# broadinstitute/permutect

Measured on AMD Instinct MI355X. Metric: read-sets/sec (train fwd+bwd), higher is better.
Workload: dtype f32 (fp32 accumulate; fwd: 2 x f16 pieces per operand = 23 bits; bwd: 2 x bf16 pieces = 16 bits)

## Files before the change

### include/permutect_amd.h

```cpp
#ifndef PERMUTECT_AMD_H
#define PERMUTECT_AMD_H

#include <stddef.h>
#include <stdint.h>

#ifdef __cplusplus
extern "C" {
#endif

#define PMT_ABI_VERSION 11

#define PMT_FAULT_JOIN 1
#define PMT_FAULT_F16_RANGE 2
#define PMT_FAULT_PLAN 4

#define PMT_OK 0
#define PMT_E_INVALID (-1)
#define PMT_E_UNSUPPORTED (-2)
#define PMT_E_CAPACITY (-3)
#define PMT_E_LAUNCH (-4)
#define PMT_E_WORKSPACE (-5)

#ifndef PMT_MAX_WIDTH
#define PMT_MAX_WIDTH 64
#endif
// ... 192 lines not shown
#define PMT_PHI_LOG_SOFTMAX 3
#define PMT_PHI_ORTHOGONAL 4
#define PMT_MAX_PHI_SEGS 48
#define PMT_MAX_ORTHO_DIM 32
typedef struct PmtPhiSeg {
    int32_t kind, theta_off, phi_off, rows, cols, reserved;
    float p0, p1;
    int32_t base_rs, base_cs;
    const float* base;
} PmtPhiSeg;
typedef struct PmtPhiProgram {
    int32_t n_segs, reserved;
    PmtPhiSeg seg[PMT_MAX_PHI_SEGS];
} PmtPhiProgram;

int pmt_phi_forward(const PmtPhiProgram* prog, const float* theta, float* phi, void* stream);
int pmt_phi_backward(const PmtPhiProgram* prog, const float* theta, const float* phi, const float* grad_phi,
                     float* grad_theta, void* stream);

typedef struct PmtIntColumn {
    const void* ptr;
    int64_t stride;
    int32_t elem_bytes, reserved;
} PmtIntColumn;

typedef struct PmtBinning {
    int32_t num_sources, num_variant_types, num_ref_bins, num_alt_bins, count_bin_skip, max_ref_count, max_alt_count, reserved;
} PmtBinning;

typedef struct PmtDownsample {
    int32_t num_variants;
// ... 32 lines not shown
    const int64_t* labels;
    int64_t label_stride;
    const int64_t* alt_counts;
    int64_t alt_count_stride;
    const int64_t* sources;
    int64_t source_stride;
    const float* weights;
    const float* source_weights;
} PmtLossArgs;
typedef struct PmtLossOutputs {
    float* supervised_b;
    float* unsupervised_b;
    float* alt_count_b;
    float* source_b;
    float* total_b;
} PmtLossOutputs;
typedef struct PmtLossInputGrads {
    float* d_logits_b;
    float* d_logits_bk;
    float* d_alt_count_raw;
    float* d_source_logits;
} PmtLossInputGrads;
int pmt_losses_forward(const PmtLossArgs* args, const PmtLossOutputs* out, void* stream);
int pmt_losses_backward(const PmtLossArgs* args, const PmtLossOutputs* grad_out, const PmtLossInputGrads* grad_in, void* stream);

typedef struct PmtRecordArgs {
    int32_t num_variants, num_bins;
    int32_t num_variant_types, num_ref_bins, num_alt_bins, count_bin_skip, max_ref_count, max_alt_count;
    PmtIntColumn labels, variant_types, sources, ref_counts, alt_counts;
    const float* weights;
// ... 136 lines not shown
```

### permutect_amd/architecture/artifact_model.py

```python
from __future__ import annotations

from typing import Optional

import torch
from torch import Tensor, nn

from permutect_amd import constants
from permutect_amd.architecture import modules as M
from permutect_amd.data.batch import Batch
from permutect_amd.data.datum import Data
from permutect_amd.engine import lib as L
from permutect_amd.engine.runtime import (HaplotypeCnnFunction, LossesFunction, PhiFunction, ReadSetEngine, ReadSetFunction,
                                          RowsMlpFunction, VariantEmbedFunction)
from permutect_amd.enums import Epoch
from permutect_amd.parameters import ModelParameters, install_pickle_alias

_BCE = nn.BCEWithLogitsLoss(reduction="none")


def gpu_if_available() -> torch.device:
    return torch.device("cuda" if torch.cuda.is_available() else "cpu")


class BatchOutput:

    def __init__(self, features_be: Tensor, ref_features_be: Tensor, logits_b: Tensor, logits_bk: Tensor,
                 weights: Tensor, source_weights: Tensor):
        self.features_be = features_be
        self.ref_features_be = ref_features_be
        self.logits_b = logits_b
        self.logits_bk = logits_bk
        self.weights = weights
        self.source_weights = source_weights

    @property
    def artifact_probs_b(self) -> Tensor:
        return torch.sigmoid(self.logits_b)

    @property
    def outlier_binary_logits(self) -> Tensor:
        lk = self.logits_bk
        nonoutlier = torch.logsumexp(torch.cat((lk[:, 0:1], lk[:, 2:]), dim=-1), dim=-1)
        return lk[:, 1] - nonoutlier


class BatchLosses:

    def __init__(self, supervised_losses_b, unsupervised_losses_b, alt_count_losses_b, source_prediction_losses_b,
                 total_losses_b):
        self.supervised_losses_b = supervised_losses_b
        self.unsupervised_losses_b = unsupervised_losses_b
        self.alt_count_losses_b = alt_count_losses_b
        self.source_prediction_losses_b = source_prediction_losses_b
        self.total_losses_b = total_losses_b
        self.total_loss = torch.sum(total_losses_b)


class SetMeansView:

    def __init__(self, means_be: Tensor, lengths_b: Tensor):
        self._means, self.lengths_b = means_be, lengths_b

    def means_over_sets(self) -> Tensor:
        return self._means

    def batch_size(self) -> int:
        return len(self.lengths_b)


class ArtifactModel(nn.Module):
# ... 97 lines not shown
            eng.pack(phi.detach().contiguous())
            eng.packed_for = (key, phi.detach()) if (key is not None and not torch.is_grad_enabled()) else None
        variant_embed = self.variant_embedding(batch)
        outs = ReadSetFunction.apply(eng, batch, phi, variant_embed)
        return outs, variant_embed

    def calculate_features(self, batch: Batch, weight_range: float = 0):
        (logits_b, logits_bk, feats, ref_feats), ve = self._encode(batch)
        e_hap = self.haplotypes_cnn.output_dimension()
        return (SetMeansView(ref_feats, batch.get(Data.REF_COUNT)), SetMeansView(feats, batch.get(Data.ALT_COUNT)),
                ve[:, ve.shape[1] - e_hap:])

    def compute_batch_output(self, batch: Batch, balancer=None) -> BatchOutput:
        (logits_b, logits_bk, feats, ref_feats), _ = self._encode(batch)
        if balancer is None:
            weights_b = source_weights = torch.ones_like(logits_b)
        elif logits_b.is_cuda and hasattr(balancer, "weights_from_logits"):
            weights_b, source_weights = balancer.weights_from_logits(batch, logits_b)
        else:
            weights_b, source_weights_b = balancer.process_batch_and_compute_weights(
                batch, artifact_probs_b=torch.sigmoid(logits_b).detach())
            source_weights = weights_b * source_weights_b
        return BatchOutput(features_be=feats, ref_features_be=ref_feats, logits_b=logits_b, logits_bk=logits_bk,
                           weights=weights_b, source_weights=source_weights)

    def compute_source_prediction_losses(self, features_be: Tensor, batch: Batch) -> Tensor:
        if self.num_sources > 1:
            eng = self.engine()
            logits = RowsMlpFunction.apply(eng, L.ROWS_SOURCE, features_be, eng.trigger,
                                           float(self.source_predictor.gradient_reversal.alpha))
            probs = torch.softmax(logits, dim=-1)
# ... 6 lines not shown
        raw = RowsMlpFunction.apply(eng, L.ROWS_ALT_COUNT, features_be, eng.trigger,
                                    float(self.alt_count_predictor.gradient_reversal.alpha))
        pred = torch.sigmoid(raw.view(-1))
        target = batch.get(Data.ALT_COUNT).to(dtype=pred.dtype) / constants.MAX_ALT_COUNT
        return self.alt_count_loss_func(pred, target)

    def compute_batch_losses(self, output: BatchOutput, batch: Batch) -> BatchLosses:
        eng = self.engine()
        alt_raw = RowsMlpFunction.apply(eng, L.ROWS_ALT_COUNT, output.features_be, eng.trigger,
                                        float(self.alt_count_predictor.gradient_reversal.alpha))
        source_logits, sources = None, None
        if self.num_sources > 1:
            source_logits = RowsMlpFunction.apply(eng, L.ROWS_SOURCE, output.features_be, eng.trigger,
                                                  float(self.source_predictor.gradient_reversal.alpha))
            sources = batch.get(Data.SOURCE).long()
        sup, unsup, alt, src, total = LossesFunction.apply(
            eng, output.logits_b, output.logits_bk, alt_raw, source_logits, batch.get(Data.LABEL).long(),
            batch.get(Data.ALT_COUNT).long(), sources, output.weights, output.source_weights)
        return BatchLosses(sup, unsup, alt, src, total)

    def compute_batch_losses_torch(self, output: BatchOutput, batch: Batch) -> BatchLosses:
        labels_b = batch.get_training_labels()
        is_labeled_b = batch.get_is_labeled_mask()
        supervised = is_labeled_b * _BCE(output.logits_b, labels_b)
        clipped = torch.clip(output.outlier_binary_logits, max=constants.MAX_OUTLIER_LOGIT)
        unsupervised = (1 - is_labeled_b) * _BCE(clipped, torch.zeros_like(clipped))
        alt_count = self.compute_alt_count_losses(output.features_be, batch)
        source = self.compute_source_prediction_losses(output.features_be, batch)
        total = output.weights * (supervised + unsupervised + alt_count) + output.source_weights * source
        return BatchLosses(supervised, unsupervised, alt_count, source, total)

    def make_dict_for_saving(self, artifact_log_priors=None, artifact_spectra=None):
        state = {k: v.detach().clone() for k, v in self.state_dict().items()}
        return {
# ... 28 lines not shown
```

### permutect_amd/csrc/pmt_losses.hip

```cpp
#include <hip/hip_runtime.h>
#include <math.h>

#include "permutect_amd.h"

#define LOSS_THREADS 256

__device__ __forceinline__ float softplus_f(float x) { return fmaxf(x, 0.f) + log1pf(expf(-fabsf(x))); }
__device__ __forceinline__ float sigmoid_f(float x) { return 1.0f / (1.0f + expf(-x)); }

struct OutlierLogit {
    float o;
    float mx, se;
};
__device__ __forceinline__ OutlierLogit outlier_logit(const float* __restrict__ lk, int K) {
    OutlierLogit r;
    r.mx = lk[0];
    for (int k = 0; k < K; ++k) r.mx = fmaxf(r.mx, lk[2 + k]);
    r.se = expf(lk[0] - r.mx);
    for (int k = 0; k < K; ++k) r.se += expf(lk[2 + k] - r.mx);
    r.o = lk[1] - (r.mx + logf(r.se));
    return r;
}

__global__ __launch_bounds__(LOSS_THREADS) void pmt_losses_forward_kernel(PmtLossArgs a, PmtLossOutputs out) {
    const int b = blockIdx.x * LOSS_THREADS + threadIdx.x;
    if (b >= a.num_variants) return;
    const int K = a.num_clusters, S = a.num_sources;
    const long long label = a.labels[(size_t)b * a.label_stride];
    const float is_labeled = label != 2 ? 1.f : 0.f;
    const float target = label == 0 ? 1.f : (label == 2 ? 0.5f : 0.f);
    const float x = a.logits_b[b];
    const float sup = is_labeled * (fmaxf(x, 0.f) - x * target + log1pf(expf(-fabsf(x))));
    const OutlierLogit ol = outlier_logit(a.logits_bk + (size_t)b * (K + 2), K);
    const float unsup = (1.f - is_labeled) * softplus_f(fminf(ol.o, a.max_outlier_logit));
    const float pred = sigmoid_f(a.alt_count_raw[b]);
    const float tgt = (float)a.alt_counts[(size_t)b * a.alt_count_stride] / a.max_alt_count;
    const float altl = (pred - tgt) * (pred - tgt);
    float src = 0.f;
    if (S > 1 && a.source_logits != nullptr) {
        const float* sl = a.source_logits + (size_t)b * S;
        const long long sid = a.sources[(size_t)b * a.source_stride];
        float mx = sl[0];
        for (int s = 1; s < S; ++s) mx = fmaxf(mx, sl[s]);
        float se = 0.f;
        for (int s = 0; s < S; ++s) se += expf(sl[s] - mx);
        for (int s = 0; s < S; ++s) {
            const float d = expf(sl[s] - mx) / se - (s == sid ? 1.f : 0.f);
            src += d * d;
        }
    }
    out.supervised_b[b] = sup;
    out.unsupervised_b[b] = unsup;
    out.alt_count_b[b] = altl;
    out.source_b[b] = src;
    out.total_b[b] = a.weights[b] * (sup + unsup + altl) + a.source_weights[b] * src;
}

__global__ __launch_bounds__(LOSS_THREADS) void pmt_losses_backward_kernel(PmtLossArgs a, PmtLossOutputs g, PmtLossInputGrads d) {
    const int b = blockIdx.x * LOSS_THREADS + threadIdx.x;
    if (b >= a.num_variants) return;
    const int K = a.num_clusters, S = a.num_sources;
    const float gt = g.total_b ? g.total_b[b] : 0.f;
    const float g_sup = (g.supervised_b ? g.supervised_b[b] : 0.f) + gt * a.weights[b];
    const float g_unsup = (g.unsupervised_b ? g.unsupervised_b[b] : 0.f) + gt * a.weights[b];
    const float g_alt = (g.alt_count_b ? g.alt_count_b[b] : 0.f) + gt * a.weights[b];
    const float g_src = (g.source_b ? g.source_b[b] : 0.f) + gt * a.source_weights[b];
    const long long label = a.labels[(size_t)b * a.label_stride];
    const float is_labeled = label != 2 ? 1.f : 0.f;
    const float target = label == 0 ? 1.f : (label == 2 ? 0.5f : 0.f);
    d.d_logits_b[b] = g_sup * is_labeled * (sigmoid_f(a.logits_b[b]) - target);
    const float* lk = a.logits_bk + (size_t)b * (K + 2);
    float* dlk = d.d_logits_bk + (size_t)b * (K + 2);
    const OutlierLogit ol = outlier_logit(lk, K);
    const float go = ol.o <= a.max_outlier_logit ? g_unsup * (1.f - is_labeled) * sigmoid_f(ol.o) : 0.f;
    dlk[1] = go;
    dlk[0] = -go * expf(lk[0] - ol.mx) / ol.se;
    for (int k = 0; k < K; ++k) dlk[2 + k] = -go * expf(lk[2 + k] - ol.mx) / ol.se;
    const float pred = sigmoid_f(a.alt_count_raw[b]);
    const float tgt = (float)a.alt_counts[(size_t)b * a.alt_count_stride] / a.max_alt_count;
    d.d_alt_count_raw[b] = g_alt * 2.f * (pred - tgt) * pred * (1.f - pred);
    if (S > 1 && a.source_logits != nullptr && d.d_source_logits != nullptr) {
// ... 7 lines not shown
        float dot = 0.f;
        for (int s = 0; s < S; ++s) {
            const float p = expf(sl[s] - mx) / se;
            dot += 2.f * (p - (s == sid ? 1.f : 0.f)) * p;
        }
        for (int s = 0; s < S; ++s) {
            const float p = expf(sl[s] - mx) / se;
            dsl[s] = g_src * (2.f * (p - (s == sid ? 1.f : 0.f)) * p - p * dot);
        }
    }
}

static int loss_args_check(const PmtLossArgs* a) {
    if (!a || a->num_variants < 0 || a->num_clusters < 0 || a->num_clusters > PMT_MAX_CLUSTERS || a->num_sources < 1) return PMT_E_INVALID;
    if (a->num_variants == 0) return PMT_OK;
    if (!a->logits_b || !a->logits_bk || !a->alt_count_raw || !a->labels || !a->alt_counts || !a->weights || !a->source_weights)
        return PMT_E_INVALID;
    if (a->num_sources > 1 && a->source_logits && !a->sources) return PMT_E_INVALID;
    return PMT_OK;
}

extern "C" int pmt_losses_forward(const PmtLossArgs* args, const PmtLossOutputs* out, void* stream) {
    const int rc = loss_args_check(args);
    if (rc) return rc;
    if (!out || !out->supervised_b || !out->unsupervised_b || !out->alt_count_b || !out->source_b || !out->total_b) return PMT_E_INVALID;
    if (args->num_variants == 0) return PMT_OK;
    hipLaunchKernelGGL(pmt_losses_forward_kernel, dim3((args->num_variants + LOSS_THREADS - 1) / LOSS_THREADS), dim3(LOSS_THREADS), 0,
                       reinterpret_cast<hipStream_t>(stream), *args, *out);
    return hipGetLastError() == hipSuccess ? PMT_OK : PMT_E_LAUNCH;
}

extern "C" int pmt_losses_backward(const PmtLossArgs* args, const PmtLossOutputs* grad_out, const PmtLossInputGrads* grad_in,
                                   void* stream) {
    const int rc = loss_args_check(args);
    if (rc) return rc;
    if (!grad_out || !grad_in || !grad_in->d_logits_b || !grad_in->d_logits_bk || !grad_in->d_alt_count_raw) return PMT_E_INVALID;
    if (args->num_variants == 0) return PMT_OK;
    hipLaunchKernelGGL(pmt_losses_backward_kernel, dim3((args->num_variants + LOSS_THREADS - 1) / LOSS_THREADS), dim3(LOSS_THREADS), 0,
                       reinterpret_cast<hipStream_t>(stream), *args, *grad_out, *grad_in);
    return hipGetLastError() == hipSuccess ? PMT_OK : PMT_E_LAUNCH;
}
// ... 89 lines not shown
```

### permutect_amd/csrc/pmt_phi.hip

```cpp
#include <hip/hip_runtime.h>
#include <math.h>

#include "permutect_amd.h"

#define PHI_THREADS 256
#define PHI_MAXN (2 * PMT_MAX_ORTHO_DIM)

__device__ double block_max(double v, double* red) {
    const int tid = threadIdx.x;
    red[tid] = v;
    __syncthreads();
    for (int s = PHI_THREADS / 2; s > 0; s >>= 1) {
        if (tid < s) red[tid] = fmax(red[tid], red[tid + s]);
        __syncthreads();
    }
    const double r = red[0];
    __syncthreads();
    return r;
}
__device__ double block_sum(double v, double* red) {
    const int tid = threadIdx.x;
    red[tid] = v;
    __syncthreads();
    for (int s = PHI_THREADS / 2; s > 0; s >>= 1) {
        if (tid < s) red[tid] += red[tid + s];
        __syncthreads();
    }
    const double r = red[0];
    __syncthreads();
    return r;
}

__device__ void matmul(double* __restrict__ Cm, const double* __restrict__ A, const double* __restrict__ B, int N, double scale) {
    for (int idx = threadIdx.x; idx < N * N; idx += PHI_THREADS) {
        const int i = idx / N, j = idx - i * N;
        double a0 = 0.0, a1 = 0.0, a2 = 0.0, a3 = 0.0;
        const double* ar = A + i * N;
        const double* bc = B + j;
        int k = 0;
        for (; k + 3 < N; k += 4) {
            a0 += ar[k] * bc[k * N];
            a1 += ar[k + 1] * bc[(k + 1) * N];
            a2 += ar[k + 2] * bc[(k + 2) * N];
            a3 += ar[k + 3] * bc[(k + 3) * N];
        }
        for (; k < N; ++k) a0 += ar[k] * bc[k * N];
        Cm[idx] = ((a0 + a1) + (a2 + a3)) * scale;
    }
    __syncthreads();
}

__device__ void expm_inplace(double* S, double* B, double* P, double* T, int N, double* red) {
    double colsum = 0.0;
    if (threadIdx.x < N)
        for (int i = 0; i < N; ++i) colsum += fabs(S[i * N + threadIdx.x]);
    const double norm1 = block_max(colsum, red);
    int s = 0;
    if (norm1 > 0.5) s = (int)ceil(log2(norm1 / 0.5));
    const double scale = ldexp(1.0, -s);
    for (int idx = threadIdx.x; idx < N * N; idx += PHI_THREADS) {
        const double b = S[idx] * scale;
        B[idx] = b;
        P[idx] = b;
        const int i = idx / N, j = idx - i * N;
        S[idx] = b + (i == j ? 1.0 : 0.0);
    }
    __syncthreads();
    for (int k = 2; k <= 12; ++k) {
        matmul(T, P, B, N, 1.0 / (double)k);
        for (int idx = threadIdx.x; idx < N * N; idx += PHI_THREADS) {
            P[idx] = T[idx];
            S[idx] += T[idx];
        }
        __syncthreads();
    }
    for (int q = 0; q < s; ++q) {
        matmul(T, S, S, N, 1.0);
        for (int idx = threadIdx.x; idx < N * N; idx += PHI_THREADS) S[idx] = T[idx];
        __syncthreads();
    }
}

struct PhiShared {
    double m[4][PHI_MAXN * PHI_MAXN];
    double red[PHI_THREADS];
};
static_assert(sizeof(PhiShared) <= 160 * 1024, "LDS budget");

__global__ __launch_bounds__(PHI_THREADS) void pmt_phi_forward_kernel(PmtPhiProgram prog, const float* __restrict__ theta,
                                                                       float* __restrict__ phi) {
    __shared__ __attribute__((aligned(16))) PhiShared sh;
    const PmtPhiSeg sg = prog.seg[blockIdx.x];
    const float* x = theta + sg.theta_off;
    float* y = phi + sg.phi_off;
    const int tid = threadIdx.x, n = sg.rows * sg.cols;
    if (sg.kind == PMT_PHI_EXP) {
        for (int i = tid; i < n; i += PHI_THREADS) y[i] = expf(x[i]);
    } else if (sg.kind == PMT_PHI_BOUNDED) {
        for (int i = tid; i < n; i += PHI_THREADS) y[i] = sg.p1 * (1.0f / (1.0f + expf(-x[i]))) + sg.p0;
    } else if (sg.kind == PMT_PHI_UNIT_ROWS) {
        for (int r = 0; r < sg.rows; ++r) {
            double q = 0.0;
            for (int i = tid; i < sg.cols; i += PHI_THREADS) q += (double)x[r * sg.cols + i] * (double)x[r * sg.cols + i];
            const float norm = (float)sqrt(block_sum(q, sh.red));
            for (int i = tid; i < sg.cols; i += PHI_THREADS) y[r * sg.cols + i] = x[r * sg.cols + i] / norm;
        }
    } else if (sg.kind == PMT_PHI_LOG_SOFTMAX) {
        for (int r = 0; r < sg.rows; ++r) {
            double mx = -INFINITY;
            for (int i = tid; i < sg.cols; i += PHI_THREADS) mx = fmax(mx, (double)x[r * sg.cols + i]);
            mx = block_max(mx, sh.red);
            double se = 0.0;
            for (int i = tid; i < sg.cols; i += PHI_THREADS) se += exp((double)x[r * sg.cols + i] - mx);
            const double lse = mx + log(block_sum(se, sh.red));
            for (int i = tid; i < sg.cols; i += PHI_THREADS) y[r * sg.cols + i] = (float)((double)x[r * sg.cols + i] - lse);
        }
    } else if (sg.kind == PMT_PHI_ORTHOGONAL) {
        const int N = sg.rows;
        double* S = sh.m[0];
        for (int idx = tid; idx < N * N; idx += PHI_THREADS) {
            const int i = idx / N, j = idx - i * N;
            S[idx] = i > j ? (double)x[i * N + j] : (i < j ? -(double)x[j * N + i] : 0.0);
        }
        __syncthreads();
        expm_inplace(S, sh.m[1], sh.m[2], sh.m[3], N, sh.red);
        for (int idx = tid; idx < N * N; idx += PHI_THREADS) {
            const int i = idx / N, j = idx - i * N;
            double acc = 0.0;
            if (sg.base != nullptr) {
                for (int k = 0; k < N; ++k) acc += (double)sg.base[i * sg.base_rs + k * sg.base_cs] * S[k * N + j];
            } else {
                acc = S[idx];
            }
            y[idx] = (float)acc;
        }
    }
}

__global__ __launch_bounds__(PHI_THREADS) void pmt_phi_backward_kernel(PmtPhiProgram prog, const float* __restrict__ theta,
                                                                        const float* __restrict__ phi,
                                                                        const float* __restrict__ gphi,
                                                                        float* __restrict__ gtheta) {
    __shared__ __attribute__((aligned(16))) PhiShared sh;
    const PmtPhiSeg sg = prog.seg[blockIdx.x];
    const float* x = theta + sg.theta_off;
    const float* y = phi + sg.phi_off;
    const float* gy = gphi + sg.phi_off;
// ... 41 lines not shown
            G[idx] = acc;
        }
        __syncthreads();
        for (int idx = tid; idx < N * N; idx += PHI_THREADS) {
            const int i = idx / N, j = idx - i * N;
            const int bi = i % nn, bj = j % nn;
            double v = 0.0;
            if ((i < nn) == (j < nn)) {
                v = bi > bj ? -(double)x[bi * nn + bj] : (bi < bj ? (double)x[bj * nn + bi] : 0.0);
            } else if (i < nn) {
                v = G[bi * nn + bj];
            }
            S[idx] = v;
        }
        __syncthreads();
        double* B = sh.m[1];
        expm_inplace(S, B, sh.m[2], sh.m[3], N, sh.red);
        for (int idx = tid; idx < nn * nn; idx += PHI_THREADS) {
            const int i = idx / nn, j = idx - i * nn;
            if (i > j) gx[idx] += (float)(S[i * N + nn + j] - S[j * N + nn + i]);
        }
    }
}

static int phi_check(const PmtPhiProgram* p) {
    if (!p || p->n_segs < 0 || p->n_segs > PMT_MAX_PHI_SEGS) return PMT_E_INVALID;
    for (int i = 0; i < p->n_segs; ++i) {
        const PmtPhiSeg* s = &p->seg[i];
        if (s->kind < PMT_PHI_EXP || s->kind > PMT_PHI_ORTHOGONAL || s->rows < 1 || s->cols < 1 || s->theta_off < 0 || s->phi_off < 0)
            return PMT_E_INVALID;
        if (s->kind == PMT_PHI_ORTHOGONAL && (s->rows != s->cols || s->rows > PMT_MAX_ORTHO_DIM)) return PMT_E_UNSUPPORTED;
    }
    return PMT_OK;
}

extern "C" int pmt_phi_forward(const PmtPhiProgram* prog, const float* theta, float* phi, void* stream) {
    const int rc = phi_check(prog);
    if (rc) return rc;
    if (!theta || !phi) return PMT_E_INVALID;
    if (prog->n_segs == 0) return PMT_OK;
    hipLaunchKernelGGL(pmt_phi_forward_kernel, dim3(prog->n_segs), dim3(PHI_THREADS), 0, reinterpret_cast<hipStream_t>(stream),
                       *prog, theta, phi);
    return hipGetLastError() == hipSuccess ? PMT_OK : PMT_E_LAUNCH;
}

extern "C" int pmt_phi_backward(const PmtPhiProgram* prog, const float* theta, const float* phi, const float* grad_phi,
                                float* grad_theta, void* stream) {
    const int rc = phi_check(prog);
    if (rc) return rc;
    if (!theta || !phi || !grad_phi || !grad_theta) return PMT_E_INVALID;
    if (prog->n_segs == 0) return PMT_OK;
    hipLaunchKernelGGL(pmt_phi_backward_kernel, dim3(prog->n_segs), dim3(PHI_THREADS), 0, reinterpret_cast<hipStream_t>(stream),
                       *prog, theta, phi, grad_phi, grad_theta);
    return hipGetLastError() == hipSuccess ? PMT_OK : PMT_E_LAUNCH;
}
```

### permutect_amd/engine/lib.py

```python
from __future__ import annotations

import ctypes as C
import os

_HERE = os.path.dirname(os.path.dirname(os.path.abspath(__file__)))
LIB_PATH = os.environ.get("PMT_LIB", os.path.join(_HERE, "libpermutect_amd.so"))

ABI_VERSION = 11
MAX_WIDTH, MAX_HALF_FFN, MAX_CLUSTERS = 64, 16, 16
MAX_HALF_FFN_WIDE = 32
MAX_WIDTH_WIDE = 128
MAX_ROW_INPUT = 128
MAX_CNN_TAPS = 192
ROWS_INFO, ROWS_ALT_COUNT, ROWS_SOURCE = 0, 1, 2
MAX_OPS, MAX_SKIP_LAYERS, MAX_BLOCKS, MAX_LINEAR = 8, 4, 16, 96
GROUP_WAVES = int(os.environ.get("PMT_GROUP_WAVES", 8))
GROUP_TILES, GROUP_MAX_SETS, TILE = 2 * GROUP_WAVES, 8 * GROUP_WAVES, 16
READS_PACKED_U8, READS_F16, READS_F32 = 0, 1, 2
OP_LINEAR, OP_SKIP = 0, 1
SLOT_FLOATS = 4 * 256

STEP_ON_DEVICE, STEP_SLOT = -1, 1000
E_INVALID, E_UNSUPPORTED, E_CAPACITY, E_LAUNCH, E_WORKSPACE = -1, -2, -3, -4, -5
_ERR = {-1: "invalid argument/descriptor", -2: "configuration not supported by the gfx950 kernels",
# ... 136 lines not shown
                ("num_alt_bins", i32), ("count_bin_skip", i32), ("max_ref_count", i32), ("max_alt_count", i32),
                ("labels", PmtIntColumn), ("variant_types", PmtIntColumn), ("sources", PmtIntColumn), ("ref_counts", PmtIntColumn),
                ("alt_counts", PmtIntColumn), ("weights", vp), ("source_weights", vp),
                ("supervised_b", vp), ("unsupervised_b", vp), ("alt_count_b", vp), ("source_b", vp)]


class PmtLossArgs(C.Structure):
    _fields_ = [("num_variants", i32), ("num_clusters", i32), ("num_sources", i32), ("reserved", i32),
                ("max_outlier_logit", C.c_float), ("max_alt_count", C.c_float),
                ("logits_b", vp), ("logits_bk", vp), ("alt_count_raw", vp), ("source_logits", vp),
                ("labels", vp), ("label_stride", i64), ("alt_counts", vp), ("alt_count_stride", i64),
                ("sources", vp), ("source_stride", i64), ("weights", vp), ("source_weights", vp)]


class PmtLossOutputs(C.Structure):
    _fields_ = [("supervised_b", vp), ("unsupervised_b", vp), ("alt_count_b", vp), ("source_b", vp), ("total_b", vp)]


class PmtLossInputGrads(C.Structure):
    _fields_ = [("d_logits_b", vp), ("d_logits_bk", vp), ("d_alt_count_raw", vp), ("d_source_logits", vp)]


EXPORTS = ["pmt_abi_version", "pmt_build_id", "pmt_shape_info", "pmt_shape_id", "pmt_limits", "pmt_struct_bytes", "pmt_model_check", "pmt_plan_groups", "pmt_plan_groups_device", "pmt_plan_device_chunks", "pmt_stash_bytes", "pmt_pack_params",
           "pmt_scan_counts", "pmt_forward", "pmt_backward", "pmt_clip_adamw",
           "pmt_dropout_mask", "pmt_rows_stash_bytes", "pmt_rows_forward", "pmt_rows_backward", "pmt_rows_workspace_floats", "pmt_cnn_forward", "pmt_cnn_backward", "pmt_cnn_stash_floats", "pmt_cnn_workspace_floats",
           "pmt_phi_forward", "pmt_phi_backward", "pmt_build_read_index", "pmt_losses_forward", "pmt_losses_backward",
           "pmt_downsample_counts", "pmt_downsample_index", "pmt_downsample_fit", "pmt_record_losses", "pmt_record_evaluation", "pmt_balance_step", "pmt_posterior_rows",
           "pmt_plan_groups_split", "pmt_layered_scratch_floats", "pmt_forward_layered",
           "pmt_layered_backward_scratch_floats", "pmt_backward_layered", "pmt_host_copy", "pmt_pack_order", "pmt_pack_order_batches", "pmt_prepare_chunk", "pmt_host_copy_rows", "pmt_compose_batch", "pmt_compose_batch_planned"]

_lib = None
# ... 60 lines not shown
    lib.pmt_pack_order.argtypes = [vp, vp, i32, i32, vp]
    lib.pmt_pack_order_batches.argtypes = [vp, vp, i32, i32, i32, i32, vp]
    lib.pmt_prepare_chunk.argtypes = [vp, i64, i32, i32, i32, i32, C.c_uint64, i32, i32, i32, vp, vp, vp, vp, i64, vp, vp]
    lib.pmt_layered_backward_scratch_floats.argtypes = [P(PmtModel), i64, i32]
    lib.pmt_layered_backward_scratch_floats.restype = C.c_size_t
    lib.pmt_backward_layered.argtypes = [P(PmtModel), vp, vp, vp, vp, P(PmtBatch), P(PmtOutputs), P(PmtOutputGrads), vp, vp, vp,
                                         vp, vp, vp, i32, vp]
    lib.pmt_downsample_counts.argtypes = [P(PmtDownsample), vp, vp, vp, vp, vp]
    lib.pmt_downsample_index.argtypes = [P(PmtDownsample), vp, vp, vp, vp, vp, vp]
    lib.pmt_downsample_fit.argtypes = [vp, i32, vp, vp, vp, vp, i32, C.c_double, C.c_double, C.c_double, C.c_double, C.c_double, vp, vp]
    lib.pmt_balance_step.argtypes = [P(PmtBalanceArgs), vp]
    lib.pmt_record_evaluation.argtypes = [P(PmtEvalArgs), vp, vp]
    lib.pmt_posterior_rows.argtypes = [vp, i64, i32, i32, vp, vp, i32, vp, i32, vp, i64, vp]
    lib.pmt_losses_forward.argtypes = [P(PmtLossArgs), P(PmtLossOutputs), vp]
    lib.pmt_losses_backward.argtypes = [P(PmtLossArgs), P(PmtLossOutputs), P(PmtLossInputGrads), vp]
    lib.pmt_phi_forward.argtypes = [P(PmtPhiProgram), vp, vp, vp]
    lib.pmt_phi_backward.argtypes = [P(PmtPhiProgram), vp, vp, vp, vp, vp]
    for name in EXPORTS:
        fn = getattr(lib, name)
        if name not in ("pmt_abi_version", "pmt_stash_bytes", "pmt_rows_stash_bytes", "pmt_layered_scratch_floats",
                        "pmt_layered_backward_scratch_floats", "pmt_cnn_stash_floats", "pmt_cnn_workspace_floats",
                        "pmt_rows_workspace_floats"):
            fn.restype = i32
    lib.pmt_struct_bytes.argtypes = [i32]
    if lib.pmt_abi_version() != ABI_VERSION:
        raise PmtError("libpermutect_amd.so ABI version mismatch; rebuild it")
    for which, st in enumerate([PmtModel, PmtBatch, PmtOutputs, PmtOutputGrads, PmtAdamW, PmtLinear, PmtOp, PmtMlp,
                                PmtBlock, PmtHead, PmtPhiProgram, PmtLossArgs, PmtDownsample, PmtRecordArgs, PmtBalanceArgs, PmtEvalArgs]):
        if lib.pmt_struct_bytes(which) != C.sizeof(st):
            raise PmtError(f"ctypes layout of {st.__name__} ({C.sizeof(st)} B) does not match the library "
                           f"({lib.pmt_struct_bytes(which)} B)")
# ... 35 lines not shown
```

### permutect_amd/engine/runtime.py

```python
from __future__ import annotations

import ctypes as C
import os
from typing import Optional, Tuple

import torch
from torch import Tensor

from permutect_amd.engine import lib as L
from permutect_amd.engine.plan import EnginePlan, ParamSpace


def _ptr(t: Optional[Tensor]) -> Optional[int]:
    return None if t is None else t.data_ptr()


def _stream() -> int:
    return L.raw_stream()


class ReadSetEngine:
    def __init__(self, model, device: torch.device):
        if device.type != "cuda":
            raise L.PmtError("permutect_amd computes on an MI355X (ROCm device 'cuda') only; there is no CPU fallback. "
                             "Model construction, state_dict and save/load work on any device.")
        self.device = device
        self.space = ParamSpace(model, device)
        self.plan = EnginePlan(model, self.space, device)
        self.lib = self.plan.lib
        self.shape_id = int(self.lib.pmt_shape_id(C.byref(self.plan.desc)))
        self._trigger = torch.zeros(1, dtype=torch.float32, device=device, requires_grad=True)
        self._no_trigger = torch.zeros(1, dtype=torch.float32, device=device)
        self._cnn_ws = None
        self._rows_ws = None
        self.join_layered = os.environ.get("PMT_LAYERED_JOIN", "1") != "0"
        self.dropout_seed = 0
        self.join_fault = torch.zeros(1, dtype=torch.int32, device=device)
        self._param_epoch = 0
        self.packed_for = None
        self.timers = None
        self.timer_stride, self._timer_calls = 1, {}
        self.grad_hook = None

    def _event_start(self, name: str):
        if self.timers is None:
            return None
        n = self._timer_calls.get(name, 0)
        self._timer_calls[name] = n + 1
        if n % max(1, int(self.timer_stride)) != 0:
# ... 54 lines not shown

    def cnn_workspace(self) -> Optional[Tensor]:
        if self._cnn_ws is None:
            n = self.lib.pmt_cnn_workspace_floats(C.byref(self.plan.desc)) if os.environ.get("PMT_CNN_WORKSPACE", "1") != "0" else 0
            self._cnn_ws = torch.empty(n, dtype=torch.float32, device=self.device) if n > 0 else False
        return self._cnn_ws if self._cnn_ws is not False else None

    def rows_workspace(self) -> Optional[Tensor]:
        if self._rows_ws is None:
            n = 0
            if os.environ.get("PMT_ROWS_WORKSPACE", "1") != "0":
                n = max(self.lib.pmt_rows_workspace_floats(C.byref(self.plan.desc), w) if self.plan.desc.row_mlp[w].n_ops > 0 else 0
                        for w in range(3))
            self._rows_ws = torch.zeros(n, dtype=torch.float32, device=self.device) if n > 0 else False
        return self._rows_ws if self._rows_ws is not False else None

    def offsets(self, batch) -> Tuple[Tensor, Tensor]:
        if getattr(batch, "_offsets", None) is None:
            ref_c, alt_c, elem, stride = batch.device_counts()
            b = batch.size()
            ref_off = torch.empty(b + 1, dtype=torch.int32, device=self.device)
            alt_off = torch.empty(b + 1, dtype=torch.int32, device=self.device)
            L.check(self.lib.pmt_scan_counts(ref_c.data_ptr(), alt_c.data_ptr(), elem, stride, b, ref_off.data_ptr(),
                                             alt_off.data_ptr(), _stream()), "pmt_scan_counts")
            batch._offsets = (ref_off, alt_off)
        return batch._offsets

    @property
    def trigger(self) -> Tensor:
        return self._trigger if torch.is_grad_enabled() else self._no_trigger
# ... 89 lines not shown

class LossesFunction(torch.autograd.Function):

    @staticmethod
    def _args(engine, logits_b, logits_bk, alt_raw, source_logits, labels, alt_counts, sources, weights, source_weights):
        from permutect_amd import constants
        a = L.PmtLossArgs()
        a.num_variants, a.num_clusters = logits_b.shape[0], logits_bk.shape[1] - 2
        a.num_sources = 1 if source_logits is None else source_logits.shape[1]
        a.max_outlier_logit, a.max_alt_count = constants.MAX_OUTLIER_LOGIT, float(constants.MAX_ALT_COUNT)
        a.logits_b, a.logits_bk, a.alt_count_raw = logits_b.data_ptr(), logits_bk.data_ptr(), alt_raw.data_ptr()
        a.source_logits = _ptr(source_logits)
        a.labels, a.label_stride = labels.data_ptr(), labels.stride(0)
        a.alt_counts, a.alt_count_stride = alt_counts.data_ptr(), alt_counts.stride(0)
        a.sources, a.source_stride = _ptr(sources), (0 if sources is None else sources.stride(0))
        a.weights, a.source_weights = weights.data_ptr(), source_weights.data_ptr()
        return a

    @staticmethod
    def forward(ctx, engine, logits_b, logits_bk, alt_raw, source_logits, labels, alt_counts, sources, weights, source_weights):
        alt_shape = alt_raw.shape
        logits_b, logits_bk, alt_raw = logits_b.contiguous(), logits_bk.contiguous(), alt_raw.contiguous().view(-1)
        source_logits = None if source_logits is None else source_logits.contiguous()
        weights, source_weights = weights.contiguous().float(), source_weights.contiguous().float()
        assert labels.dtype == torch.int64 and alt_counts.dtype == torch.int64 and (sources is None or sources.dtype == torch.int64)
        b = logits_b.shape[0]
        outs = [torch.empty(b, dtype=torch.float32, device=logits_b.device) for _ in range(5)]
        a = LossesFunction._args(engine, logits_b, logits_bk, alt_raw, source_logits, labels, alt_counts, sources, weights, source_weights)
        o = L.PmtLossOutputs(*[t.data_ptr() for t in outs])
        L.check(engine.lib.pmt_losses_forward(C.byref(a), C.byref(o), _stream()), "pmt_losses_forward")
        ctx.engine = engine
        ctx.alt_shape = alt_shape
        ctx.set_materialize_grads(False)
        ctx.save_for_backward(logits_b, logits_bk, alt_raw, labels, alt_counts, weights, source_weights,
                              *(() if source_logits is None else (source_logits, sources)))
        return tuple(outs)

    @staticmethod
    def backward(ctx, *grads):
        saved = ctx.saved_tensors
        logits_b, logits_bk, alt_raw, labels, alt_counts, weights, source_weights = saved[:7]
        source_logits, sources = (saved[7], saved[8]) if len(saved) > 7 else (None, None)
        grads = [None if g is None else g.contiguous().float() for g in grads]
        a = LossesFunction._args(ctx.engine, logits_b, logits_bk, alt_raw, source_logits, labels, alt_counts, sources, weights, source_weights)
        g = L.PmtLossOutputs(*[_ptr(t) for t in grads])
        d_b, d_bk, d_alt = torch.empty_like(logits_b), torch.empty_like(logits_bk), torch.empty_like(alt_raw)
        d_src = None if source_logits is None else torch.empty_like(source_logits)
        d = L.PmtLossInputGrads(d_b.data_ptr(), d_bk.data_ptr(), d_alt.data_ptr(), _ptr(d_src))
        L.check(ctx.engine.lib.pmt_losses_backward(C.byref(a), C.byref(g), C.byref(d), _stream()), "pmt_losses_backward")
        return None, d_b, d_bk, d_alt.view(ctx.alt_shape), d_src, None, None, None, None, None


class PhiFunction(torch.autograd.Function):

    @staticmethod
    def forward(ctx, engine: "ReadSetEngine", prog, trigger: Tensor):
        phi = torch.zeros(engine.plan.desc.phi_size, dtype=torch.float32, device=engine.device)
        L.check(engine.lib.pmt_phi_forward(C.byref(prog), engine.space.theta.data_ptr(), phi.data_ptr(), _stream()), "pmt_phi_forward")
        ctx.engine, ctx.prog = engine, prog
        ctx.save_for_backward(phi)
        return phi

    @staticmethod
    def backward(ctx, gphi: Tensor):
        (phi,) = ctx.saved_tensors
        eng = ctx.engine
        gphi = gphi.contiguous()
        L.check(eng.lib.pmt_phi_backward(C.byref(ctx.prog), eng.space.theta.data_ptr(), phi.data_ptr(), gphi.data_ptr(),
                                         eng.space.gtheta.data_ptr(), _stream()), "pmt_phi_backward")
        return None, None, None


class ReadSetFunction(torch.autograd.Function):
# ... 170 lines not shown
```

Measured before the change: 19.41 million.

## Fuse loss sum into loss kernel, drop unit weights, speed up matrix exponential

The loss forward kernel now also computes the total loss through block reductions and a last-block-done ticket, which replaces a separate torch.sum launch. Unit weight tensors are no longer allocated when there is no balancer; the kernels treat null weights as 1. The phi kernel zeroes its own uncovered tail instead of needing a separate torch.zeros fill, uses 512 threads, and evaluates the degree-12 Taylor series for the matrix exponential with a Paterson–Stockmeyer style split, cutting the number of matrix multiplies. The aim is fewer launches and less work per step, at the cost of atomic-counter state, more complex code, and a changed ABI.

```diff
diff --git a/include/permutect_amd.h b/include/permutect_amd.h
--- a/include/permutect_amd.h
+++ b/include/permutect_amd.h
@@ -8,7 +8,7 @@
 extern "C" {
 #endif
 
-#define PMT_ABI_VERSION 11
+#define PMT_ABI_VERSION 12
 
 #define PMT_FAULT_JOIN 1
 #define PMT_FAULT_F16_RANGE 2
@@ -231,7 +231,7 @@
     PmtPhiSeg seg[PMT_MAX_PHI_SEGS];
 } PmtPhiProgram;
 
-int pmt_phi_forward(const PmtPhiProgram* prog, const float* theta, float* phi, void* stream);
+int pmt_phi_forward(const PmtPhiProgram* prog, const float* theta, float* phi, int32_t phi_size, void* stream);
 int pmt_phi_backward(const PmtPhiProgram* prog, const float* theta, const float* phi, const float* grad_phi,
                      float* grad_theta, void* stream);
 
@@ -294,6 +294,9 @@
     float* alt_count_b;
     float* source_b;
     float* total_b;
+    float* total;
+    float* total_partials;
+    int32_t* total_counter;
 } PmtLossOutputs;
 typedef struct PmtLossInputGrads {
     float* d_logits_b;
diff --git a/permutect_amd/architecture/artifact_model.py b/permutect_amd/architecture/artifact_model.py
--- a/permutect_amd/architecture/artifact_model.py
+++ b/permutect_amd/architecture/artifact_model.py
@@ -33,6 +33,17 @@
         self.weights = weights
         self.source_weights = source_weights
 
+    def _ones(self) -> Tensor:
+        if self._unit is None:
+            self._unit = torch.ones_like(self.logits_b)
+        return self._unit
+
+    _unit = None
+    weights = property(lambda self: self._ones() if self._weights is None else self._weights,
+                       lambda self, w: setattr(self, "_weights", w))
+    source_weights = property(lambda self: self._ones() if self._source_weights is None else self._source_weights,
+                              lambda self, w: setattr(self, "_source_weights", w))
+
     @property
     def artifact_probs_b(self) -> Tensor:
         return torch.sigmoid(self.logits_b)
@@ -47,13 +58,13 @@
 class BatchLosses:
 
     def __init__(self, supervised_losses_b, unsupervised_losses_b, alt_count_losses_b, source_prediction_losses_b,
-                 total_losses_b):
+                 total_losses_b, total_loss=None):
         self.supervised_losses_b = supervised_losses_b
         self.unsupervised_losses_b = unsupervised_losses_b
         self.alt_count_losses_b = alt_count_losses_b
         self.source_prediction_losses_b = source_prediction_losses_b
         self.total_losses_b = total_losses_b
-        self.total_loss = torch.sum(total_losses_b)
+        self.total_loss = torch.sum(total_losses_b) if total_loss is None else total_loss
 
 
 class SetMeansView:
@@ -181,7 +192,7 @@
     def compute_batch_output(self, batch: Batch, balancer=None) -> BatchOutput:
         (logits_b, logits_bk, feats, ref_feats), _ = self._encode(batch)
         if balancer is None:
-            weights_b = source_weights = torch.ones_like(logits_b)
+            weights_b = source_weights = None
         elif logits_b.is_cuda and hasattr(balancer, "weights_from_logits"):
             weights_b, source_weights = balancer.weights_from_logits(batch, logits_b)
         else:
@@ -218,10 +229,10 @@
             source_logits = RowsMlpFunction.apply(eng, L.ROWS_SOURCE, output.features_be, eng.trigger,
                                                   float(self.source_predictor.gradient_reversal.alpha))
             sources = batch.get(Data.SOURCE).long()
-        sup, unsup, alt, src, total = LossesFunction.apply(
+        sup, unsup, alt, src, total, total_sum = LossesFunction.apply(
             eng, output.logits_b, output.logits_bk, alt_raw, source_logits, batch.get(Data.LABEL).long(),
-            batch.get(Data.ALT_COUNT).long(), sources, output.weights, output.source_weights)
-        return BatchLosses(sup, unsup, alt, src, total)
+            batch.get(Data.ALT_COUNT).long(), sources, output._weights, output._source_weights)
+        return BatchLosses(sup, unsup, alt, src, total, total_loss=total_sum)
 
     def compute_batch_losses_torch(self, output: BatchOutput, batch: Batch) -> BatchLosses:
         labels_b = batch.get_training_labels()
diff --git a/permutect_amd/csrc/pmt_losses.hip b/permutect_amd/csrc/pmt_losses.hip
--- a/permutect_amd/csrc/pmt_losses.hip
+++ b/permutect_amd/csrc/pmt_losses.hip
@@ -22,9 +22,7 @@
     return r;
 }
 
-__global__ __launch_bounds__(LOSS_THREADS) void pmt_losses_forward_kernel(PmtLossArgs a, PmtLossOutputs out) {
-    const int b = blockIdx.x * LOSS_THREADS + threadIdx.x;
-    if (b >= a.num_variants) return;
+__device__ __forceinline__ float losses_of_variant(const PmtLossArgs& a, const PmtLossOutputs& out, int b) {
     const int K = a.num_clusters, S = a.num_sources;
     const long long label = a.labels[(size_t)b * a.label_stride];
     const float is_labeled = label != 2 ? 1.f : 0.f;
@@ -53,18 +51,57 @@
     out.unsupervised_b[b] = unsup;
     out.alt_count_b[b] = altl;
     out.source_b[b] = src;
-    out.total_b[b] = a.weights[b] * (sup + unsup + altl) + a.source_weights[b] * src;
+    const float w = a.weights ? a.weights[b] : 1.f, sw = a.source_weights ? a.source_weights[b] : 1.f;
+    const float total = w * (sup + unsup + altl) + sw * src;
+    out.total_b[b] = total;
+    return total;
+}
+
+__device__ __forceinline__ double loss_block_sum(double v, double* red) {
+    red[threadIdx.x] = v;
+    __syncthreads();
+    for (int s = LOSS_THREADS / 2; s > 0; s >>= 1) {
+        if (threadIdx.x < s) red[threadIdx.x] += red[threadIdx.x + s];
+        __syncthreads();
+    }
+    return red[0];
+}
+
+__global__ __launch_bounds__(LOSS_THREADS) void pmt_losses_forward_kernel(PmtLossArgs a, PmtLossOutputs out) {
+    __shared__ double red[LOSS_THREADS + 1];
+    const int b = blockIdx.x * LOSS_THREADS + threadIdx.x;
+    const float total = b < a.num_variants ? losses_of_variant(a, out, b) : 0.f;
+    if (out.total == nullptr) return;
+    const double part = loss_block_sum((double)total, red);
+    if (threadIdx.x == 0) {
+        __hip_atomic_store(&out.total_partials[blockIdx.x], (float)part, __ATOMIC_RELAXED, __HIP_MEMORY_SCOPE_AGENT);
+        asm volatile("s_waitcnt vmcnt(0)" ::: "memory");
+        const int ticket = __hip_atomic_fetch_add(out.total_counter, 1, __ATOMIC_RELAXED, __HIP_MEMORY_SCOPE_AGENT);
+        red[LOSS_THREADS] = ticket == (int)gridDim.x - 1 ? 1.0 : 0.0;
+    }
+    __syncthreads();
+    if (red[LOSS_THREADS] == 0.0) return;
+    __syncthreads();
+    double acc = 0.0;
+    for (int i = threadIdx.x; i < (int)gridDim.x; i += LOSS_THREADS)
+        acc += (double)__hip_atomic_load(&out.total_partials[i], __ATOMIC_RELAXED, __HIP_MEMORY_SCOPE_AGENT);
+    const double sum = loss_block_sum(acc, red);
+    if (threadIdx.x == 0) {
+        *out.total = (float)sum;
+        __hip_atomic_store(out.total_counter, 0, __ATOMIC_RELAXED, __HIP_MEMORY_SCOPE_AGENT);
+    }
 }
 
 __global__ __launch_bounds__(LOSS_THREADS) void pmt_losses_backward_kernel(PmtLossArgs a, PmtLossOutputs g, PmtLossInputGrads d) {
     const int b = blockIdx.x * LOSS_THREADS + threadIdx.x;
     if (b >= a.num_variants) return;
     const int K = a.num_clusters, S = a.num_sources;
-    const float gt = g.total_b ? g.total_b[b] : 0.f;
-    const float g_sup = (g.supervised_b ? g.supervised_b[b] : 0.f) + gt * a.weights[b];
-    const float g_unsup = (g.unsupervised_b ? g.unsupervised_b[b] : 0.f) + gt * a.weights[b];
-    const float g_alt = (g.alt_count_b ? g.alt_count_b[b] : 0.f) + gt * a.weights[b];
-    const float g_src = (g.source_b ? g.source_b[b] : 0.f) + gt * a.source_weights[b];
+    const float gt = g.total_b ? (g.total ? g.total_b[b] + *g.total : g.total_b[b]) : (g.total ? *g.total : 0.f);
+    const float w = a.weights ? a.weights[b] : 1.f, sw = a.source_weights ? a.source_weights[b] : 1.f;
+    const float g_sup = (g.supervised_b ? g.supervised_b[b] : 0.f) + gt * w;
+    const float g_unsup = (g.unsupervised_b ? g.unsupervised_b[b] : 0.f) + gt * w;
+    const float g_alt = (g.alt_count_b ? g.alt_count_b[b] : 0.f) + gt * w;
+    const float g_src = (g.source_b ? g.source_b[b] : 0.f) + gt * sw;
     const long long label = a.labels[(size_t)b * a.label_stride];
     const float is_labeled = label != 2 ? 1.f : 0.f;
     const float target = label == 0 ? 1.f : (label == 2 ? 0.5f : 0.f);
@@ -102,8 +139,7 @@
 static int loss_args_check(const PmtLossArgs* a) {
     if (!a || a->num_variants < 0 || a->num_clusters < 0 || a->num_clusters > PMT_MAX_CLUSTERS || a->num_sources < 1) return PMT_E_INVALID;
     if (a->num_variants == 0) return PMT_OK;
-    if (!a->logits_b || !a->logits_bk || !a->alt_count_raw || !a->labels || !a->alt_counts || !a->weights || !a->source_weights)
-        return PMT_E_INVALID;
+    if (!a->logits_b || !a->logits_bk || !a->alt_count_raw || !a->labels || !a->alt_counts) return PMT_E_INVALID;
     if (a->num_sources > 1 && a->source_logits && !a->sources) return PMT_E_INVALID;
     return PMT_OK;
 }
@@ -112,7 +148,9 @@
     const int rc = loss_args_check(args);
     if (rc) return rc;
     if (!out || !out->supervised_b || !out->unsupervised_b || !out->alt_count_b || !out->source_b || !out->total_b) return PMT_E_INVALID;
-    if (args->num_variants == 0) return PMT_OK;
+    if (out->total && (!out->total_partials || !out->total_counter)) return PMT_E_INVALID;
+    if (args->num_variants == 0)
+        return !out->total || hipMemsetAsync(out->total, 0, sizeof(float), reinterpret_cast<hipStream_t>(stream)) == hipSuccess ? PMT_OK : PMT_E_LAUNCH;
     hipLaunchKernelGGL(pmt_losses_forward_kernel, dim3((args->num_variants + LOSS_THREADS - 1) / LOSS_THREADS), dim3(LOSS_THREADS), 0,
                        reinterpret_cast<hipStream_t>(stream), *args, *out);
     return hipGetLastError() == hipSuccess ? PMT_OK : PMT_E_LAUNCH;
diff --git a/permutect_amd/csrc/pmt_phi.hip b/permutect_amd/csrc/pmt_phi.hip
--- a/permutect_amd/csrc/pmt_phi.hip
+++ b/permutect_amd/csrc/pmt_phi.hip
@@ -3,7 +3,7 @@
 
 #include "permutect_amd.h"
 
-#define PHI_THREADS 256
+#define PHI_THREADS 512
 #define PHI_MAXN (2 * PMT_MAX_ORTHO_DIM)
 
 __device__ double block_max(double v, double* red) {
@@ -31,54 +31,109 @@
     return r;
 }
 
-__device__ void matmul(double* __restrict__ Cm, const double* __restrict__ A, const double* __restrict__ B, int N, double scale) {
-    for (int idx = threadIdx.x; idx < N * N; idx += PHI_THREADS) {
-        const int i = idx / N, j = idx - i * N;
-        double a0 = 0.0, a1 = 0.0, a2 = 0.0, a3 = 0.0;
-        const double* ar = A + i * N;
-        const double* bc = B + j;
-        int k = 0;
-        for (; k + 3 < N; k += 4) {
-            a0 += ar[k] * bc[k * N];
-            a1 += ar[k + 1] * bc[(k + 1) * N];
-            a2 += ar[k + 2] * bc[(k + 2) * N];
-            a3 += ar[k + 3] * bc[(k + 3) * N];
-        }
-        for (; k < N; ++k) a0 += ar[k] * bc[k * N];
-        Cm[idx] = ((a0 + a1) + (a2 + a3)) * scale;
-    }
-    __syncthreads();
-}
-
-__device__ void expm_inplace(double* S, double* B, double* P, double* T, int N, double* red) {
-    double colsum = 0.0;
-    if (threadIdx.x < N)
-        for (int i = 0; i < N; ++i) colsum += fabs(S[i * N + threadIdx.x]);
-    const double norm1 = block_max(colsum, red);
+struct PhiWalk {
+    int N, di, dj, i0, j0;
+    __device__ explicit PhiWalk(int n) : N(n), di(PHI_THREADS / n), dj(PHI_THREADS % n), i0((int)threadIdx.x / n), j0((int)threadIdx.x % n) {}
+    __device__ void next(int& i, int& j) const {
+        i += di;
+        j += dj;
+        if (j >= N) {
+            j -= N;
+            ++i;
+        }
+    }
+};
+
+__device__ __forceinline__ double phi_dot(const double* __restrict__ ar, const double* __restrict__ bc, int N) {
+    double a0 = 0.0, a1 = 0.0, a2 = 0.0, a3 = 0.0;
+    int k = 0;
+    for (; k + 3 < N; k += 4) {
+        a0 += ar[k] * bc[k * N];
+        a1 += ar[k + 1] * bc[(k + 1) * N];
+        a2 += ar[k + 2] * bc[(k + 2) * N];
+        a3 += ar[k + 3] * bc[(k + 3) * N];
+    }
+    for (; k < N; ++k) a0 += ar[k] * bc[k * N];
+    return (a0 + a1) + (a2 + a3);
+}
+
+__device__ void matmul(double* __restrict__ Cm, const double* __restrict__ A, const double* __restrict__ B, const PhiWalk& w, double scale,
+                       const double* __restrict__ D = nullptr) {
+    const int N = w.N;
+    for (int idx = threadIdx.x, i = w.i0, j = w.j0; idx < N * N; idx += PHI_THREADS, w.next(i, j)) {
+        const double v = phi_dot(A + i * N, B + j, N) * scale;
+        Cm[idx] = D != nullptr ? D[idx] + v : v;
+    }
+    __syncthreads();
+}
+
+#define PHI_POOL (4 * PHI_MAXN * PHI_MAXN)
+#define PHI_PS_MATS 6
+
+__device__ double* expm_pool(double* pool, int N, double* red) {
+    const int NN = N * N, tid = threadIdx.x;
+    double* S = pool;
+    if (tid < N) {
+        double colsum = 0.0;
+        for (int i = 0; i < N; ++i) colsum += fabs(S[i * N + tid]);
+        red[tid] = colsum;
+    }
+    __syncthreads();
+    double norm1 = 0.0;
+    for (int j = 0; j < N; ++j) norm1 = fmax(norm1, red[j]);
     int s = 0;
     if (norm1 > 0.5) s = (int)ceil(log2(norm1 / 0.5));
     const double scale = ldexp(1.0, -s);
-    for (int idx = threadIdx.x; idx < N * N; idx += PHI_THREADS) {
-        const double b = S[idx] * scale;
-        B[idx] = b;
-        P[idx] = b;
-        const int i = idx / N, j = idx - i * N;
-        S[idx] = b + (i == j ? 1.0 : 0.0);
-    }
-    __syncthreads();
-    for (int k = 2; k <= 12; ++k) {
-        matmul(T, P, B, N, 1.0 / (double)k);
-        for (int idx = threadIdx.x; idx < N * N; idx += PHI_THREADS) {
-            P[idx] = T[idx];
-            S[idx] += T[idx];
-        }
-        __syncthreads();
+    const PhiWalk w(N);
+    double *R, *T;
+    if (PHI_PS_MATS * NN <= PHI_POOL) {
+        double *B = S, *B2 = pool + NN, *B4 = pool + 2 * NN, *Q0 = pool + 3 * NN, *Q1 = pool + 4 * NN, *Q2 = pool + 5 * NN;
+        for (int idx = tid; idx < NN; idx += PHI_THREADS) B[idx] *= scale;
+        __syncthreads();
+        matmul(B2, B, B, w, 1.0);
+        constexpr double c2 = 1.0 / 2, c3 = 1.0 / 6, c4 = 1.0 / 24, c5 = 1.0 / 120, c6 = 1.0 / 720, c7 = 1.0 / 5040, c8 = 1.0 / 40320,
+                         c9 = 1.0 / 362880, c10 = 1.0 / 3628800, c11 = 1.0 / 39916800, c12 = 1.0 / 479001600;
+        for (int idx = tid, i = w.i0, j = w.j0; idx < NN; idx += PHI_THREADS, w.next(i, j)) {
+            const double b3 = phi_dot(B2 + i * N, B + j, N), b4 = phi_dot(B2 + i * N, B2 + j, N);
+            const double b1 = B[idx], b2 = B2[idx], eye = i == j ? 1.0 : 0.0;
+            B4[idx] = b4;
+            Q0[idx] = eye + b1 + c2 * b2 + c3 * b3;
+            Q1[idx] = c4 * eye + c5 * b1 + c6 * b2 + c7 * b3;
+            Q2[idx] = c8 * eye + c9 * b1 + c10 * b2 + c11 * b3 + c12 * b4;
+        }
+        __syncthreads();
+        double* U = B;
+        matmul(U, B4, Q2, w, 1.0, Q1);
+        R = B2;
+        matmul(R, B4, U, w, 1.0, Q0);
+        T = U;
+    } else {
+        double *B = pool + PHI_MAXN * PHI_MAXN, *P = pool + 2 * PHI_MAXN * PHI_MAXN;
+        T = pool + 3 * PHI_MAXN * PHI_MAXN;
+        for (int idx = tid, i = w.i0, j = w.j0; idx < NN; idx += PHI_THREADS, w.next(i, j)) {
+            const double b = S[idx] * scale;
+            B[idx] = b;
+            P[idx] = b;
+            S[idx] = b + (i == j ? 1.0 : 0.0);
+        }
+        __syncthreads();
+        for (int k = 2; k <= 12; ++k) {
+            matmul(T, P, B, w, 1.0 / (double)k);
+            for (int idx = tid; idx < NN; idx += PHI_THREADS) {
+                P[idx] = T[idx];
+                S[idx] += T[idx];
+            }
+            __syncthreads();
+        }
+        R = S;
     }
     for (int q = 0; q < s; ++q) {
-        matmul(T, S, S, N, 1.0);
-        for (int idx = threadIdx.x; idx < N * N; idx += PHI_THREADS) S[idx] = T[idx];
-        __syncthreads();
-    }
+        matmul(T, R, R, w, 1.0);
+        double* t = R;
+        R = T;
+        T = t;
+    }
+    return R;
 }
 
 struct PhiShared {
@@ -88,12 +143,14 @@
 static_assert(sizeof(PhiShared) <= 160 * 1024, "LDS budget");
 
 __global__ __launch_bounds__(PHI_THREADS) void pmt_phi_forward_kernel(PmtPhiProgram prog, const float* __restrict__ theta,
-                                                                       float* __restrict__ phi) {
+                                                                       float* __restrict__ phi, int phi_covered, int phi_size) {
     __shared__ __attribute__((aligned(16))) PhiShared sh;
     const PmtPhiSeg sg = prog.seg[blockIdx.x];
     const float* x = theta + sg.theta_off;
     float* y = phi + sg.phi_off;
     const int tid = threadIdx.x, n = sg.rows * sg.cols;
+    if (blockIdx.x == 0)
+        for (int i = phi_covered + tid; i < phi_size; i += PHI_THREADS) phi[i] = 0.f;
     if (sg.kind == PMT_PHI_EXP) {
         for (int i = tid; i < n; i += PHI_THREADS) y[i] = expf(x[i]);
     } else if (sg.kind == PMT_PHI_BOUNDED) {
@@ -123,14 +180,14 @@
             S[idx] = i > j ? (double)x[i * N + j] : (i < j ? -(double)x[j * N + i] : 0.0);
         }
         __syncthreads();
-        expm_inplace(S, sh.m[1], sh.m[2], sh.m[3], N, sh.red);
+        const double* Q = expm_pool(S, N, sh.red);
         for (int idx = tid; idx < N * N; idx += PHI_THREADS) {
             const int i = idx / N, j = idx - i * N;
             double acc = 0.0;
             if (sg.base != nullptr) {
-                for (int k = 0; k < N; ++k) acc += (double)sg.base[i * sg.base_rs + k * sg.base_cs] * S[k * N + j];
+                for (int k = 0; k < N; ++k) acc += (double)sg.base[i * sg.base_rs + k * sg.base_cs] * Q[k * N + j];
             } else {
-                acc = S[idx];
+                acc = Q[idx];
             }
             y[idx] = (float)acc;
         }
@@ -202,11 +259,10 @@
             S[idx] = v;
         }
         __syncthreads();
-        double* B = sh.m[1];
-        expm_inplace(S, B, sh.m[2], sh.m[3], N, sh.red);
+        const double* E = expm_pool(S, N, sh.red);
         for (int idx = tid; idx < nn * nn; idx += PHI_THREADS) {
             const int i = idx / nn, j = idx - i * nn;
-            if (i > j) gx[idx] += (float)(S[i * N + nn + j] - S[j * N + nn + i]);
+            if (i > j) gx[idx] += (float)(E[i * N + nn + j] - E[j * N + nn + i]);
         }
     }
 }
@@ -222,13 +278,22 @@
     return PMT_OK;
 }
 
-extern "C" int pmt_phi_forward(const PmtPhiProgram* prog, const float* theta, float* phi, void* stream) {
+extern "C" int pmt_phi_forward(const PmtPhiProgram* prog, const float* theta, float* phi, int32_t phi_size, void* stream) {
     const int rc = phi_check(prog);
     if (rc) return rc;
-    if (!theta || !phi) return PMT_E_INVALID;
-    if (prog->n_segs == 0) return PMT_OK;
+    if (!theta || !phi || phi_size < 0) return PMT_E_INVALID;
+    int covered = 0, sum = 0;
+    for (int i = 0; i < prog->n_segs; ++i) {
+        const int size = prog->seg[i].rows * prog->seg[i].cols, end = prog->seg[i].phi_off + size;
+        if (end > phi_size) return PMT_E_INVALID;
+        if (end > covered) covered = end;
+        sum += size;
+    }
+    if (sum != covered) return PMT_E_UNSUPPORTED;
+    if (prog->n_segs == 0)
+        return hipMemsetAsync(phi, 0, sizeof(float) * (size_t)phi_size, reinterpret_cast<hipStream_t>(stream)) == hipSuccess ? PMT_OK : PMT_E_LAUNCH;
     hipLaunchKernelGGL(pmt_phi_forward_kernel, dim3(prog->n_segs), dim3(PHI_THREADS), 0, reinterpret_cast<hipStream_t>(stream),
-                       *prog, theta, phi);
+                       *prog, theta, phi, covered, (int)phi_size);
     return hipGetLastError() == hipSuccess ? PMT_OK : PMT_E_LAUNCH;
 }
 
diff --git a/permutect_amd/engine/lib.py b/permutect_amd/engine/lib.py
--- a/permutect_amd/engine/lib.py
+++ b/permutect_amd/engine/lib.py
@@ -6,7 +6,7 @@
 _HERE = os.path.dirname(os.path.dirname(os.path.abspath(__file__)))
 LIB_PATH = os.environ.get("PMT_LIB", os.path.join(_HERE, "libpermutect_amd.so"))
 
-ABI_VERSION = 11
+ABI_VERSION = 12
 MAX_WIDTH, MAX_HALF_FFN, MAX_CLUSTERS = 64, 16, 16
 MAX_HALF_FFN_WIDE = 32
 MAX_WIDTH_WIDE = 128
@@ -174,7 +174,8 @@
 
 
 class PmtLossOutputs(C.Structure):
-    _fields_ = [("supervised_b", vp), ("unsupervised_b", vp), ("alt_count_b", vp), ("source_b", vp), ("total_b", vp)]
+    _fields_ = [("supervised_b", vp), ("unsupervised_b", vp), ("alt_count_b", vp), ("source_b", vp), ("total_b", vp),
+                ("total", vp), ("total_partials", vp), ("total_counter", vp)]
 
 
 class PmtLossInputGrads(C.Structure):
@@ -265,7 +266,7 @@
     lib.pmt_posterior_rows.argtypes = [vp, i64, i32, i32, vp, vp, i32, vp, i32, vp, i64, vp]
     lib.pmt_losses_forward.argtypes = [P(PmtLossArgs), P(PmtLossOutputs), vp]
     lib.pmt_losses_backward.argtypes = [P(PmtLossArgs), P(PmtLossOutputs), P(PmtLossInputGrads), vp]
-    lib.pmt_phi_forward.argtypes = [P(PmtPhiProgram), vp, vp, vp]
+    lib.pmt_phi_forward.argtypes = [P(PmtPhiProgram), vp, vp, i32, vp]
     lib.pmt_phi_backward.argtypes = [P(PmtPhiProgram), vp, vp, vp, vp, vp]
     for name in EXPORTS:
         fn = getattr(lib, name)
diff --git a/permutect_amd/engine/runtime.py b/permutect_amd/engine/runtime.py
--- a/permutect_amd/engine/runtime.py
+++ b/permutect_amd/engine/runtime.py
@@ -33,6 +33,7 @@
         self._no_trigger = torch.zeros(1, dtype=torch.float32, device=device)
         self._cnn_ws = None
         self._rows_ws = None
+        self._loss_ws = None
         self.join_layered = os.environ.get("PMT_LAYERED_JOIN", "1") != "0"
         self.dropout_seed = 0
         self.join_fault = torch.zeros(1, dtype=torch.int32, device=device)
@@ -117,6 +118,13 @@
                         for w in range(3))
             self._rows_ws = torch.zeros(n, dtype=torch.float32, device=self.device) if n > 0 else False
         return self._rows_ws if self._rows_ws is not False else None
+
+    def loss_workspace(self, b: int) -> Tuple[Tensor, Tensor]:
+        n = max(1, (b + 255) // 256)
+        if self._loss_ws is None or self._loss_ws[0].numel() < n:
+            counter = torch.zeros(1, dtype=torch.int32, device=self.device) if self._loss_ws is None else self._loss_ws[1]
+            self._loss_ws = (torch.empty(max(n, 512), dtype=torch.float32, device=self.device), counter)
+        return self._loss_ws
 
     def offsets(self, batch) -> Tuple[Tensor, Tensor]:
         if getattr(batch, "_offsets", None) is None:
@@ -236,7 +244,7 @@
         a.labels, a.label_stride = labels.data_ptr(), labels.stride(0)
         a.alt_counts, a.alt_count_stride = alt_counts.data_ptr(), alt_counts.stride(0)
         a.sources, a.source_stride = _ptr(sources), (0 if sources is None else sources.stride(0))
-        a.weights, a.source_weights = weights.data_ptr(), source_weights.data_ptr()
+        a.weights, a.source_weights = _ptr(weights), _ptr(source_weights)
         return a
 
     @staticmethod
@@ -244,28 +252,34 @@
         alt_shape = alt_raw.shape
         logits_b, logits_bk, alt_raw = logits_b.contiguous(), logits_bk.contiguous(), alt_raw.contiguous().view(-1)
         source_logits = None if source_logits is None else source_logits.contiguous()
-        weights, source_weights = weights.contiguous().float(), source_weights.contiguous().float()
+        weights = None if weights is None else weights.contiguous().float()
+        source_weights = None if source_weights is None else source_weights.contiguous().float()
         assert labels.dtype == torch.int64 and alt_counts.dtype == torch.int64 and (sources is None or sources.dtype == torch.int64)
         b = logits_b.shape[0]
         outs = [torch.empty(b, dtype=torch.float32, device=logits_b.device) for _ in range(5)]
         a = LossesFunction._args(engine, logits_b, logits_bk, alt_raw, source_logits, labels, alt_counts, sources, weights, source_weights)
-        o = L.PmtLossOutputs(*[t.data_ptr() for t in outs])
+        total = torch.empty((), dtype=torch.float32, device=logits_b.device)
+        partials, counter = engine.loss_workspace(b)
+        o = L.PmtLossOutputs(*[t.data_ptr() for t in outs], total.data_ptr(), partials.data_ptr(), counter.data_ptr())
         L.check(engine.lib.pmt_losses_forward(C.byref(a), C.byref(o), _stream()), "pmt_losses_forward")
         ctx.engine = engine
         ctx.alt_shape = alt_shape
+        ctx.has_weights, ctx.has_sources = weights is not None, source_logits is not None
         ctx.set_materialize_grads(False)
-        ctx.save_for_backward(logits_b, logits_bk, alt_raw, labels, alt_counts, weights, source_weights,
-                              *(() if source_logits is None else (source_logits, sources)))
-        return tuple(outs)
+        ctx.save_for_backward(logits_b, logits_bk, alt_raw, labels, alt_counts,
+                              *((weights, source_weights) if ctx.has_weights else ()),
+                              *((source_logits, sources) if ctx.has_sources else ()))
+        return (*outs, total)
 
     @staticmethod
     def backward(ctx, *grads):
-        saved = ctx.saved_tensors
-        logits_b, logits_bk, alt_raw, labels, alt_counts, weights, source_weights = saved[:7]
-        source_logits, sources = (saved[7], saved[8]) if len(saved) > 7 else (None, None)
+        saved = list(ctx.saved_tensors)
+        logits_b, logits_bk, alt_raw, labels, alt_counts = saved[:5]
+        weights, source_weights = (saved[5], saved[6]) if ctx.has_weights else (None, None)
+        source_logits, sources = (saved[-2], saved[-1]) if ctx.has_sources else (None, None)
         grads = [None if g is None else g.contiguous().float() for g in grads]
         a = LossesFunction._args(ctx.engine, logits_b, logits_bk, alt_raw, source_logits, labels, alt_counts, sources, weights, source_weights)
-        g = L.PmtLossOutputs(*[_ptr(t) for t in grads])
+        g = L.PmtLossOutputs(*[_ptr(t) for t in grads], None, None)
         d_b, d_bk, d_alt = torch.empty_like(logits_b), torch.empty_like(logits_bk), torch.empty_like(alt_raw)
         d_src = None if source_logits is None else torch.empty_like(source_logits)
         d = L.PmtLossInputGrads(d_b.data_ptr(), d_bk.data_ptr(), d_alt.data_ptr(), _ptr(d_src))
@@ -277,8 +291,9 @@
 
     @staticmethod
     def forward(ctx, engine: "ReadSetEngine", prog, trigger: Tensor):
-        phi = torch.zeros(engine.plan.desc.phi_size, dtype=torch.float32, device=engine.device)
-        L.check(engine.lib.pmt_phi_forward(C.byref(prog), engine.space.theta.data_ptr(), phi.data_ptr(), _stream()), "pmt_phi_forward")
+        phi = torch.empty(engine.plan.desc.phi_size, dtype=torch.float32, device=engine.device)
+        L.check(engine.lib.pmt_phi_forward(C.byref(prog), engine.space.theta.data_ptr(), phi.data_ptr(), phi.numel(), _stream()),
+                "pmt_phi_forward")
         ctx.engine, ctx.prog = engine, prog
         ctx.save_for_backward(phi)
         return phi
```

Measured after the change: 19.50 million (median of 6 runs). About the same (+0.5%).
